# PantoMatrix/PantoMatrix

Hardware: NVIDIA H100
Metric: motion_frames_per_sec (higher is better)
Workload: dtype fp16x3 (two fp16 operand planes, 3 products, f32 accumulate)

## Files before the change

include/pm_emage.h:

```cpp
#ifndef PM_EMAGE_H
#define PM_EMAGE_H
#include <stdint.h>
#ifdef __cplusplus
extern "C" {
#endif

#define PM_ABI_VERSION 5
#define PM_FMT_F16 0x100
#define PM_TC_TILE_SHIFT 16
int pm_abi_version(void);
int pm_memset_async(void* ptr, int value, long long bytes, void* stream);
int pm_device_cc(void);

int pm_tapgemm_f32(const float* A, long long a_bs, int lda, int batch, int rows_in, int cin,
                   const float* W, const float* bias, int taps, int stride, int pad,
                   int rows_out, int cout,
                   const float* residual, long long r_bs, int ldr,
                   int act, float slope,
                   float* out, long long o_bs, int ldo, void* stream);

int pm_tapgemm_tc(const uint16_t* A, long long a_ps, long long a_bs, int lda, int batch, int rows_in, int cin,
                  const uint16_t* W, long long w_ps, int w_rows, int ldw, int taps, int pad, int nsplit,
                  const float* bias, int rows_out, int cout,
                  const float* residual, long long r_bs, int ldr,
                  int act, int act_cols, float slope, float acc_scale,
                  float* out_f32, long long o_bs, int ldo,
                  uint16_t* out_bf16, long long ob_ps, long long ob_bs, int ldob, int out_nsplit,
                  const void* prefetch, long long prefetch_bytes, void* stream);

int pm_split_bf16(const float* x, long long x_bs, int ldx, int batch, int rows, int ch,
                  uint16_t* out, long long o_ps, long long o_bs, int ldo, int nsplit, void* stream);

int pm_wav_stem_f32(const float* audio, long long a_bs, long long a_ws, int batch, int windows, int n_samples,
                    const float* w1, const float* b1, const float* wd, const float* bd, int cout,
                    int ksize, int stride, int pad, int rows_out, float slope,
                    float* y1, float* sc,
                    uint16_t* planes, long long p_ps, int p_ld, int p_nsplit, void* stream);

int pm_add_layernorm_f32(const float* x, const float* r, const float* gamma, const float* beta,
                         float* out, long long rows, int ch, float eps,
                         uint16_t* planes, long long p_ps, int p_ld, int p_nsplit, void* stream);

int pm_attention_f32(const float* Q, int ldq, const float* K, int ldk, const float* V, int ldv,
                     float* O, int ldo, int batch, int heads, int tq, int tk, int head_dim,
                     uint16_t* planes, long long p_ps, int p_ld, int p_nsplit, void* stream);

int pm_attention_tc(const uint16_t* Q, long long q_ps, long long q_bs, int ldq, int q_cols, int q_col0,
                    const uint16_t* K, long long k_ps, long long k_bs, int ldk, int k_cols, int k_col0,
                    const uint16_t* V, long long v_ps, long long v_bs, int ldv, int v_cols, int v_col0,
                    float* O, int ldo, int batch, int heads, int tq, int tk, int head_dim,
                    uint16_t* planes, long long p_ps, int p_ld, int p_nsplit, void* stream);

int pm_add_rows_f32(const float* x, const float* pe, const float* spk, int first, int second,
                    float* out, int batch, int rows, int ch,
                    uint16_t* planes, long long p_ps, int p_ld, int p_nsplit, void* stream);
int pm_add2_f32(const float* a, const float* b, float* out, long long n, int ch,
                uint16_t* planes, long long p_ps, int p_ld, int p_nsplit, void* stream);
int pm_add2_strided_f32(const float* a, long long lda, const float* b, long long ldb, float* out, long long ldo,
                        long long rows, long long ch,
                        uint16_t* planes, long long p_ps, int p_ld, int p_nsplit, void* stream);

int pm_window_input_f32(const float* motion, const float* mask, const float* seed, const float* mask_embedding,
                        float* out, int batch, int total_len, int start, int win_len, int pre, int ch, long long seed_bs,
                        uint16_t* planes, long long p_ps, int p_ld, int p_nsplit, void* stream);

int pm_l2_argmin_f32(const float* z, long long rows, int rows_per_batch, long long z_bs,
                     const float* codebook, const float* e2, int n_codes, int e_dim, long long* index, void* stream);
int pm_l2_argmin_tc(const float* z, long long rows, int rows_per_batch, long long z_bs,
                    const float* codebook, const float* e2, int n_codes, int e_dim, long long* index, int max_ctas,
                    void* stream);
int pm_l2_argmin_simt_f32(const float* z, long long rows, int rows_per_batch, long long z_bs,
                          const float* codebook, const float* e2, int n_codes, int e_dim, long long* index, void* stream);
int pm_row_argmax_f32(const float* x, long long rows, int ch, int ldx, int rows_per_batch, long long x_bs,
                      long long* index, int* nonfinite, void* stream);
int pm_gather_rows_f32(const float* codebook, long long n_table, const long long* index, long long rows, int ch,
                       float* out, uint16_t* planes, long long p_ps, int p_ld, int p_nsplit, void* stream);
int pm_row_sqnorm_f32(const float* x, int rows, int ch, float* out, void* stream);

int pm_pose_compose_f32(const float* face, const float* upper, const float* hands, const float* lower,
                        float* expression, float* axis_angle, float* motion4inf, long long bt, void* stream);

int pm_global_trans_f32(const float* rec, int ld, int vel_off, const float* ref_trans, int ref_bs, float dt,
                        float* trans, int batch, int t, void* stream);

int pm_resample_poly_f32(const void* pcm, int is_int16, long long in_bs, int batch, long long n_in, int channels,
                         const float* bank, int up, int down, int taps, long long n_pre_remove,
                         float* out, long long out_bs, void* stream);

int pm_lstm_bidir_f32(const float* xproj, long long x_bs, int ldx, const float* whh,
                      float* y, long long y_bs, int ldy, unsigned int* barrier,
                      int batch, int t, int hidden, void* stream);
int pm_lstm_cond_f32(const float* spk, long long n_spk, int spk_dim, const long long* speaker_id,
// ... 11 lines not shown
```

pantomatrix_b200/csrc/pm_tapgemm_tc.cu:

```cuda
#include <cuda.h>
#include <stdio.h>
#include <stdlib.h>

#include <cstring>
#include "pm_common.cuh"
#include "../../include/pm_emage.h"


namespace {

constexpr int BM = 128;
constexpr int BK = 64;
constexpr int MMA_K = 16;
constexpr int A_TILE_BYTES = BM * BK * 2;
constexpr int PRODUCER_THREADS = 128;
constexpr int CONSUMER_THREADS = 256;
constexpr int NUM_THREADS = PRODUCER_THREADS + CONSUMER_THREADS;
constexpr int PRODUCER_REGS = 40, CONSUMER_REGS = 232;
static_assert(PRODUCER_THREADS * PRODUCER_REGS + CONSUMER_THREADS * CONSUMER_REGS == (65536 / NUM_THREADS & ~7) * NUM_THREADS,
              "the setmaxnreg split must use exactly the launch's register pool");
constexpr int STAMP_WARP = PRODUCER_THREADS / 32;
constexpr int MAX_STAGES = 8;
constexpr int RING_KB = 200;

struct TcParams {
  int taps, pad, nsplit, kblocks;
  int rows_out, cout, batch;
  int R, NB;
  int w_rows;
  const float* bias;
  const float* residual; long long r_bs; int ldr;
  int act, act_cols; float slope;
  float* out_f32; long long o_bs; int ldo;
  __nv_bfloat16* out_bf16; long long ob_ps, ob_bs; int ldob; int out_nsplit;
  int stages;
  const uint8_t* prefetch; long long prefetch_bytes;
  float acc_scale;
};

#ifdef PM_TC_TIMING
__device__ unsigned long long pm_tc_stamps[4096 * 8];
#define PM_STAMP(i)                                                                                              \
  do {                                                                                                           \
    if ((threadIdx.x & 31) == 0) {                                                                               \
      const unsigned cta_ = (blockIdx.z * gridDim.y + blockIdx.y) * gridDim.x + blockIdx.x;                      \
      if (cta_ < 4096) pm_tc_stamps[cta_ * 8 + (i)] = (unsigned long long)clock64();                             \
    }                                                                                                            \
  } while (0)
#else
#define PM_STAMP(i) do {} while (0)
#endif

#include "pm_tc_ptx.cuh"

template <int BN, bool F16>
__device__ __forceinline__ void mma_k16(float (&d)[BN / 2], uint64_t a, uint64_t b) {
  static_assert(BN == 64 || BN == 128, "64- or 128-column tiles (see pm_tapgemm_tc)");
  if constexpr (BN == 64) wgmma_m64n64k16<!F16>(d, a, b);
  else wgmma_m64n128k16<!F16>(d, a, b);
}

template <int BN, bool F16, int NSPLIT>
__device__ __forceinline__ void mma_kblock(float (&main)[BN / 2], float (&corr)[BN / 2], uint64_t a0, uint64_t w0) {
  constexpr uint64_t A_PL = A_TILE_BYTES >> 4, W_PL = (BN * BK * 2) >> 4, K_ST = (MMA_K * 2) >> 4;
  if constexpr (NSPLIT == 3) {
#pragma unroll
    for (int k = 0; k < BK / MMA_K; ++k) mma_k16<BN, F16>(corr, a0 + k * K_ST, w0 + 2 * W_PL + k * K_ST);
#pragma unroll
    for (int k = 0; k < BK / MMA_K; ++k) mma_k16<BN, F16>(corr, a0 + A_PL + k * K_ST, w0 + W_PL + k * K_ST);
#pragma unroll
    for (int k = 0; k < BK / MMA_K; ++k) mma_k16<BN, F16>(corr, a0 + 2 * A_PL + k * K_ST, w0 + k * K_ST);
  }
  if constexpr (NSPLIT >= 2) {
#pragma unroll
    for (int k = 0; k < BK / MMA_K; ++k) mma_k16<BN, F16>(corr, a0 + k * K_ST, w0 + W_PL + k * K_ST);
#pragma unroll
    for (int k = 0; k < BK / MMA_K; ++k) mma_k16<BN, F16>(corr, a0 + A_PL + k * K_ST, w0 + k * K_ST);
  }
#pragma unroll
  for (int k = 0; k < BK / MMA_K; ++k) mma_k16<BN, F16>(main, a0 + k * K_ST, w0 + k * K_ST);
}

template <int BN, bool F16, int NSPLIT>
__global__ void __launch_bounds__(NUM_THREADS, 1) tapgemm_tc_kernel(const __grid_constant__ CUtensorMap map_a,
                                                                  const __grid_constant__ CUtensorMap map_w,
                                                                  const TcParams p) {
  constexpr int W_TILE_BYTES = BN * BK * 2;
  constexpr int NACC = BN / 2;
  constexpr int ST = BN + 8;

  extern __shared__ __align__(1024) uint8_t smem_raw[];
  uint8_t* tiles = reinterpret_cast<uint8_t*>((reinterpret_cast<uintptr_t>(smem_raw) + 1023) & ~uintptr_t(1023));
  const int stage_bytes = p.nsplit * (A_TILE_BYTES + W_TILE_BYTES);
  const int ring_bytes = p.stages * stage_bytes > BM * ST * 4 ? p.stages * stage_bytes : BM * ST * 4;
  uint64_t* bars = reinterpret_cast<uint64_t*>(tiles + ring_bytes);
  uint64_t* full_bar = bars;
  uint64_t* empty_bar = bars + MAX_STAGES;

  const int warp = threadIdx.x >> 5, lane = threadIdx.x & 31;
  if (warp == STAMP_WARP) PM_STAMP(0);
  const int l0 = blockIdx.x * p.R;
  const int n0 = blockIdx.y * BN;
  const int b0 = blockIdx.z * p.NB;
  const int n_iter = p.taps * p.kblocks;

  if (threadIdx.x == 0) {
    asm volatile("prefetch.tensormap [%0];" ::"l"(&map_a) : "memory");
    asm volatile("prefetch.tensormap [%0];" ::"l"(&map_w) : "memory");
    for (int s = 0; s < p.stages; ++s) {
      mbar_init(smem_u32(&full_bar[s]), 1);
      mbar_init(smem_u32(&empty_bar[s]), 2);
    }
    asm volatile("fence.mbarrier_init.release.cluster;" ::: "memory");
  }
  __syncthreads();
  if (warp == STAMP_WARP) PM_STAMP(1);

  if (warp < PRODUCER_THREADS / 32) {
    setmaxnreg_dec<PRODUCER_REGS>();
    if (warp == 1 && lane == 0 && p.prefetch) {
      const long long ncta = (long long)gridDim.x * gridDim.y * gridDim.z;
      const long long cta = ((long long)blockIdx.z * gridDim.y + blockIdx.y) * gridDim.x + blockIdx.x;
      long long share = ((p.prefetch_bytes + ncta - 1) / ncta + 127) & ~127LL;
      long long off = cta * share;
      long long end = off + share < p.prefetch_bytes ? off + share : p.prefetch_bytes;
      end &= ~15LL;
      for (; off < end; off += 16384) {
        const uint32_t n = (uint32_t)(end - off < 16384 ? end - off : 16384);
        asm volatile("cp.async.bulk.prefetch.L2.global [%0], %1;" ::"l"(p.prefetch + off), "r"(n) : "memory");
      }
    }
    if (warp != 0) return;
    const uint32_t tx = (uint32_t)stage_bytes;
    int s = 0, tap = 0, kb = 0;
    uint32_t ph = 0;
    for (int it = 0; it < n_iter; ++it) {
      mbar_wait_fast(smem_u32(&empty_bar[s]), ph ^ 1u);
      if (elect_one()) {
        const uint32_t bar = smem_u32(&full_bar[s]);
        uint8_t* st = tiles + (size_t)s * stage_bytes;
        mbar_expect_tx(bar, tx);
        for (int pl = 0; pl < p.nsplit; ++pl) {
          tma_load_4d(smem_u32(st + pl * A_TILE_BYTES), &map_a, bar, kb * BK, l0 + tap - p.pad, b0, pl);
          tma_load_3d(smem_u32(st + p.nsplit * A_TILE_BYTES + pl * W_TILE_BYTES), &map_w, bar, kb * BK, tap * p.w_rows + n0, pl);
        }
      }
      __syncwarp();
      if (++s == p.stages) { s = 0; ph ^= 1u; }
      if (++kb == p.kblocks) { kb = 0; ++tap; }
    }
    return;
  }

  setmaxnreg_inc<CONSUMER_REGS>();
  const int ct = threadIdx.x - PRODUCER_THREADS;
  const int wg = ct >> 7;
  float acc0[NACC], acc1[NACC], accc[NACC];
#pragma unroll
  for (int i = 0; i < NACC; ++i) { acc0[i] = 0.f; acc1[i] = 0.f; accc[i] = 0.f; }
  {
    const uint32_t tiles_u32 = smem_u32(tiles);
    int s = 0;
    uint32_t ph = 0;
    int prev = -1;
    auto kblock = [&](float (&main)[NACC]) {
      mbar_wait_fast(smem_u32(&full_bar[s]), ph);
      if (prev < 0 && warp == STAMP_WARP) PM_STAMP(2);
      const uint32_t a_base = tiles_u32 + (uint32_t)s * (uint32_t)stage_bytes + (uint32_t)wg * (64 * 128);
      const uint32_t w_base = tiles_u32 + (uint32_t)s * (uint32_t)stage_bytes + (uint32_t)(NSPLIT * A_TILE_BYTES);
      wgmma_fence();
      mma_kblock<BN, F16, NSPLIT>(main, accc, gmma_desc(GMMA_DESC_K_SW128, a_base), gmma_desc(GMMA_DESC_K_SW128, w_base));
      wgmma_commit();
      wgmma_wait<1>();
      if (prev >= 0 && ct % 128 == 0) mbar_arrive(smem_u32(&empty_bar[prev]));
      prev = s;
      if (++s == p.stages) { s = 0; ph ^= 1u; }
    };
    int it = 0;
    for (; it + 1 < n_iter; it += 2) {
      kblock(acc0);
      kblock(acc1);
    }
    if (it < n_iter) kblock(acc0);
    if (warp == STAMP_WARP) PM_STAMP(3);
    wgmma_wait<0>();
    if (warp == STAMP_WARP) PM_STAMP(4);
    wgmma_fence_regs(acc0);
    wgmma_fence_regs(acc1);
    wgmma_fence_regs(accc);
  }
  named_bar_sync(1, CONSUMER_THREADS);
  {
    const int wq = warp & 3, t4 = lane & 3;
    const int r0 = wg * 64 + wq * 16 + (lane >> 2);
    float* stg = reinterpret_cast<float*>(tiles);
#pragma unroll
    for (int i = 0; i < NACC / 4; ++i) {
      const int c = 8 * i + 2 * t4;
#pragma unroll
      for (int h = 0; h < 2; ++h) {
        float v0 = acc0[4 * i + 2 * h] + acc1[4 * i + 2 * h];
        float v1 = acc0[4 * i + 2 * h + 1] + acc1[4 * i + 2 * h + 1];
        v0 += accc[4 * i + 2 * h];
        v1 += accc[4 * i + 2 * h + 1];
        if constexpr (F16) { v0 *= p.acc_scale; v1 *= p.acc_scale; }
        *reinterpret_cast<float2*>(stg + (r0 + 8 * h) * ST + c) = make_float2(v0, v1);
      }
    }
  }
  named_bar_sync(1, CONSUMER_THREADS);

  const bool vec_f = p.out_f32 && ((p.ldo & 3) == 0) && ((reinterpret_cast<uintptr_t>(p.out_f32) & 15) == 0) && ((p.o_bs & 3) == 0);
  const bool vec_r = p.residual && ((p.ldr & 3) == 0) && ((reinterpret_cast<uintptr_t>(p.residual) & 15) == 0) && ((p.r_bs & 3) == 0);
  const bool vec_b = p.out_bf16 && ((p.ldob & 3) == 0) && ((reinterpret_cast<uintptr_t>(p.out_bf16) & 7) == 0) &&
                     ((p.ob_bs & 3) == 0) && ((p.ob_ps & 3) == 0);
  const bool all_vec = (!p.out_f32 || vec_f) && (!p.residual || vec_r) && (!p.out_bf16 || vec_b);
  const float act_slope = p.act == PM_ACT_NONE ? 1.f : (p.act == PM_ACT_RELU ? 0.f : p.slope);
  const int r_shift = 31 - __clz(p.R);
  constexpr int C4 = BN / 4;
  const float* stg = reinterpret_cast<const float*>(tiles);
#pragma unroll 1
  for (int item = ct; item < BM * C4; item += CONSUMER_THREADS) {
    const int rt = item / C4, c = (item % C4) * 4;
    const int b = b0 + (rt >> r_shift), l = l0 + (rt & (p.R - 1));
    const int n = n0 + c;
    if (b >= p.batch || l >= p.rows_out || n >= p.cout) continue;
    const float4 x4 = *reinterpret_cast<const float4*>(stg + rt * ST + c);
    const long long of = (long long)b * p.o_bs + (long long)l * p.ldo;
    const long long orr = (long long)b * p.r_bs + (long long)l * p.ldr;
    const PmPlanes P{p.out_bf16 ? p.out_bf16 + (long long)b * p.ob_bs + (long long)l * p.ldob : nullptr,
                     p.ob_ps, p.ldob, p.out_nsplit};
    if (all_vec && n + 4 <= p.cout) {
      float4 x = x4;
      if (p.bias) { x.x += __ldg(p.bias + n); x.y += __ldg(p.bias + n + 1); x.z += __ldg(p.bias + n + 2); x.w += __ldg(p.bias + n + 3); }
      if (p.residual) {
        const float4 t = *reinterpret_cast<const float4*>(p.residual + orr + n);
        x.x += t.x; x.y += t.y; x.z += t.z; x.w += t.w;
      }
      x.x = x.x < 0.f ? (n < p.act_cols ? act_slope : 1.f) * x.x : x.x;
      x.y = x.y < 0.f ? (n + 1 < p.act_cols ? act_slope : 1.f) * x.y : x.y;
      x.z = x.z < 0.f ? (n + 2 < p.act_cols ? act_slope : 1.f) * x.z : x.z;
      x.w = x.w < 0.f ? (n + 3 < p.act_cols ? act_slope : 1.f) * x.w : x.w;
      if (p.out_f32) *reinterpret_cast<float4*>(p.out_f32 + of + n) = x;
      if (P.ptr) pm_store_planes4_t<F16>(P, 0, n, x);
    } else {
      const float xs[4] = {x4.x, x4.y, x4.z, x4.w};
#pragma unroll
      for (int k = 0; k < 4; ++k) {
        if (n + k >= p.cout) break;
        float y = xs[k];
        if (p.bias) y += __ldg(p.bias + n + k);
        if (p.residual) y += p.residual[orr + n + k];
        y = y < 0.f ? (n + k < p.act_cols ? act_slope : 1.f) * y : y;
        if (p.out_f32) p.out_f32[of + n + k] = y;
        if (P.ptr) pm_store_planes_t<F16>(P, 0, n + k, y);
      }
    }
  }
  if (warp == STAMP_WARP) PM_STAMP(5);
#ifdef PM_TC_TIMING
  named_bar_sync(1, CONSUMER_THREADS);
#endif
  if (warp == STAMP_WARP) PM_STAMP(6);
}

template <bool VEC, bool F16>
__global__ void __launch_bounds__(256) split_bf16_kernel(const float* __restrict__ x, long long x_bs, int ldx, int rows,
                                                         int ch, __nv_bfloat16* __restrict__ out, long long o_ps,
                                                         long long o_bs, int ldo, int nsplit) {
  const int b = blockIdx.y;
  const float* __restrict__ xb = x + (long long)b * x_bs;
  __nv_bfloat16* __restrict__ ob = out + (long long)b * o_bs;
  if (VEC) {
    const int ch4 = ch >> 2;
    const long long total = (long long)rows * ch4;
    for (long long i = (long long)blockIdx.x * blockDim.x + threadIdx.x; i < total; i += (long long)gridDim.x * blockDim.x) {
      const int r = (int)(i / ch4), c4 = (int)(i - (long long)r * ch4);
      const float4 v = *reinterpret_cast<const float4*>(xb + (long long)r * ldx + 4 * c4);
      const PmPlanes P{ob, o_ps, ldo, nsplit};
      pm_store_planes4_t<F16>(P, r, 4 * c4, v);
    }
  } else {
    const long long total = (long long)rows * ch;
    for (long long i = (long long)blockIdx.x * blockDim.x + threadIdx.x; i < total; i += (long long)gridDim.x * blockDim.x) {
      const int r = (int)(i / ch), c = (int)(i - (long long)r * ch);
      const PmPlanes P{ob, o_ps, ldo, nsplit};
      pm_store_planes_t<F16>(P, r, c, xb[(long long)r * ldx + c]);
    }
  }
}

template <int BN, bool F16, int NSPLIT>
int launch(const CUtensorMap& ma, const CUtensorMap& mw, TcParams& p, dim3 grid, cudaStream_t st) {
  const int stage_bytes = p.nsplit * (A_TILE_BYTES + BN * BK * 2);
  int stages = RING_KB * 1024 / stage_bytes;
  if (stages > MAX_STAGES) stages = MAX_STAGES;
  if (stages < 2) return PM_EUNSUPPORTED;
  p.stages = stages;
  const int staging = BM * (BN + 8) * 4;
  const size_t ring = (size_t)stages * stage_bytes > (size_t)staging ? (size_t)stages * stage_bytes : (size_t)staging;
  const size_t smem = ring + 1024  + 2 * MAX_STAGES * sizeof(uint64_t);
  static unsigned long long configured = 0;
  if (pm_first_use_on_device(configured)) {
    cudaError_t e = cudaFuncSetAttribute(tapgemm_tc_kernel<BN, F16, NSPLIT>, cudaFuncAttributeMaxDynamicSharedMemorySize, 227 * 1024);
    if (e != cudaSuccess) { configured = 0; return (int)e; }
  }
  tapgemm_tc_kernel<BN, F16, NSPLIT><<<grid, NUM_THREADS, smem, st>>>(ma, mw, p);
  PM_LAUNCH_CHECK();
}

template <int BN>
int launch_fmt(const CUtensorMap& ma, const CUtensorMap& mw, TcParams& p, dim3 grid, cudaStream_t st, bool f16) {
  if (f16) {
    if (p.nsplit == 1) return launch<BN, true, 1>(ma, mw, p, grid, st);
    if (p.nsplit == 2) return launch<BN, true, 2>(ma, mw, p, grid, st);
    return launch<BN, true, 3>(ma, mw, p, grid, st);
  }
  if (p.nsplit == 1) return launch<BN, false, 1>(ma, mw, p, grid, st);
  if (p.nsplit == 2) return launch<BN, false, 2>(ma, mw, p, grid, st);
  return launch<BN, false, 3>(ma, mw, p, grid, st);
}

int pick_bn(long long row_tiles, int cout, int w_rows, int sms) {
  if (cout <= 64 || w_rows % 128) return 64;
  const long long waves64 = (row_tiles * pm_cdiv(cout, 64) + sms - 1) / sms;
  const long long waves128 = (row_tiles * pm_cdiv(cout, 128) + sms - 1) / sms;
  return waves128 * 14 <= waves64 * 10 ? 128 : 64;
}

}

extern "C" int pm_tapgemm_tc(const uint16_t* A, long long a_ps, long long a_bs, int lda, int batch, int rows_in, int cin,
                             const uint16_t* W, long long w_ps, int w_rows, int ldw, int taps, int pad, int nsplit,
                             const float* bias, int rows_out, int cout,
                             const float* residual, long long r_bs, int ldr,
                             int act, int act_cols, float slope, float acc_scale,
                             float* out_f32, long long o_bs, int ldo,
                             uint16_t* out_bf16, long long ob_ps, long long ob_bs, int ldob, int out_nsplit,
                             const void* prefetch, long long prefetch_bytes, void* stream) {
  PM_REQUIRE(A && W && (out_f32 || out_bf16));
  const int tile = (nsplit >> PM_TC_TILE_SHIFT) & 0xff;
  PM_TAKE_FMT(nsplit, f16);
  PM_TAKE_FMT(out_nsplit, out_f16);
  PM_REQUIRE(!out_bf16 || out_f16 == f16);
  PM_REQUIRE(f16 || acc_scale == 1.0f);
  PM_REQUIRE(!prefetch || (prefetch_bytes >= 0 && (reinterpret_cast<uintptr_t>(prefetch) & 15) == 0));
  PM_REQUIRE(batch > 0 && rows_in > 0 && rows_out > 0 && cin > 0 && cout > 0 && taps > 0);
  PM_REQUIRE(nsplit >= 1 && nsplit <= 3 && (!out_bf16 || (out_nsplit >= 1 && out_nsplit <= 3)));
  PM_REQUIRE(act >= PM_ACT_NONE && act <= PM_ACT_LEAKY);
  PM_REQUIRE((reinterpret_cast<uintptr_t>(A) & 15) == 0 && (reinterpret_cast<uintptr_t>(W) & 15) == 0);
  PM_REQUIRE((lda & 7) == 0 && (ldw & 7) == 0 && lda >= cin && ldw >= cin && w_rows >= cout);
  PM_REQUIRE(batch == 1 || (a_bs & 7) == 0);
  PM_REQUIRE(nsplit == 1 || ((a_ps & 7) == 0 && (w_ps & 7) == 0));
  PM_REQUIRE(!out_f32 || ldo >= cout);
  PM_REQUIRE(!out_bf16 || ldob >= cout);
  PM_REQUIRE(!residual || ldr >= cout);

  int R = 128;
  if (rows_out <= 64 && batch > 1) { R = 16; while (R < rows_out) R <<= 1; }
  const int NB = 128 / R;
  PM_REQUIRE(tile <= 2 && w_rows % 64 == 0 && (tile != 2 || w_rows % 128 == 0));
  int BNsel = tile == 1 ? 64 : 128;
  if (tile == 0) {
    int dev = 0, sms = 0;
    cudaError_t e = cudaGetDevice(&dev);
    if (e == cudaSuccess) e = cudaDeviceGetAttribute(&sms, cudaDevAttrMultiProcessorCount, dev);
    if (e != cudaSuccess) return (int)e;
    BNsel = pick_bn((long long)pm_cdiv(rows_out, R) * pm_cdiv(batch, NB), cout, w_rows, sms);
  }

  TcParams p;
  p.taps = taps; p.pad = pad; p.nsplit = nsplit; p.kblocks = (cin + BK - 1) / BK;
  p.rows_out = rows_out; p.cout = cout; p.batch = batch; p.R = R; p.NB = NB; p.w_rows = w_rows;
  p.bias = bias; p.residual = residual; p.r_bs = r_bs; p.ldr = ldr;
  p.act = act; p.act_cols = act_cols <= 0 ? cout : act_cols; p.slope = slope;
  p.out_f32 = out_f32; p.o_bs = o_bs; p.ldo = ldo;
  p.out_bf16 = reinterpret_cast<__nv_bfloat16*>(out_bf16); p.ob_ps = ob_ps; p.ob_bs = ob_bs; p.ldob = ldob;
  p.out_nsplit = out_bf16 ? out_nsplit : 0;
  p.stages = 0;
  p.prefetch = static_cast<const uint8_t*>(prefetch);
  p.prefetch_bytes = prefetch ? prefetch_bytes : 0;
  p.acc_scale = acc_scale;
  CUtensorMap ma, mw;
  {
    const long long bs_el = batch > 1 ? a_bs : (long long)rows_in * lda;
    const long long ps_el = nsplit > 1 ? a_ps : bs_el * batch;
    cuuint64_t dims[4] = {(cuuint64_t)cin, (cuuint64_t)rows_in, (cuuint64_t)batch, (cuuint64_t)nsplit};
    cuuint64_t strides[3] = {(cuuint64_t)lda * 2, (cuuint64_t)bs_el * 2, (cuuint64_t)ps_el * 2};
    cuuint32_t box[4] = {(cuuint32_t)BK, (cuuint32_t)R, (cuuint32_t)NB, 1};
    if (!encode_map(&ma, A, 4, dims, strides, box, f16)) return PM_EBADARG;
  }
  {
    const long long ps_el = nsplit > 1 ? w_ps : (long long)taps * w_rows * ldw;
    cuuint64_t dims[3] = {(cuuint64_t)cin, (cuuint64_t)taps * w_rows, (cuuint64_t)nsplit};
    cuuint64_t strides[2] = {(cuuint64_t)ldw * 2, (cuuint64_t)ps_el * 2};
    cuuint32_t box[3] = {(cuuint32_t)BK, (cuuint32_t)BNsel, 1};
    if (!encode_map(&mw, W, 3, dims, strides, box, f16)) return PM_EBADARG;
  }
  dim3 grid(pm_cdiv(rows_out, R), pm_cdiv(cout, BNsel), pm_cdiv(batch, NB));
  PM_REQUIRE(grid.z <= 65535 && grid.y <= 65535);
  const cudaStream_t st = (cudaStream_t)stream;
  if (BNsel == 128) return launch_fmt<128>(ma, mw, p, grid, st, f16);
  return launch_fmt<64>(ma, mw, p, grid, st, f16);
}

#ifdef PM_TC_TIMING
extern "C" int pm_tc_timing_reset() {
  cudaError_t e = cudaDeviceSynchronize();
  if (e != cudaSuccess) return (int)e;
  void* d = nullptr;
  e = cudaGetSymbolAddress(&d, pm_tc_stamps);
  if (e != cudaSuccess) return (int)e;
  return (int)cudaMemset(d, 0, sizeof(unsigned long long) * 4096 * 8);
}
extern "C" int pm_tc_timing_read(unsigned long long* host) {
  cudaError_t e = cudaDeviceSynchronize();
  if (e != cudaSuccess) return (int)e;
  return (int)cudaMemcpyFromSymbol(host, pm_tc_stamps, sizeof(unsigned long long) * 4096 * 8);
}
#endif

extern "C" int pm_split_bf16(const float* x, long long x_bs, int ldx, int batch, int rows, int ch,
                             uint16_t* out, long long o_ps, long long o_bs, int ldo, int nsplit, void* stream) {
  PM_TAKE_FMT(nsplit, f16);
  PM_REQUIRE(x && out && batch >= 0 && rows >= 0 && ch > 0 && ldx >= ch && ldo >= ch && nsplit >= 1 && nsplit <= 3);
  if ((long long)batch * rows == 0) return PM_OK;
  PM_REQUIRE(batch <= 65535);
  const bool vec = (ch & 3) == 0 && (ldx & 3) == 0 && (x_bs & 3) == 0 && (ldo & 3) == 0 && (o_bs & 3) == 0 &&
                   (o_ps & 3) == 0 && (reinterpret_cast<uintptr_t>(x) & 15) == 0 && (reinterpret_cast<uintptr_t>(out) & 7) == 0;
  const long long work = (long long)rows * (vec ? ch / 4 : ch);
  long long gx = (work + 255) / 256;
  const long long cap = batch >= 132 * 4 ? 1 : (132 * 8 + batch - 1) / batch;
  if (gx > cap) gx = cap;
  dim3 grid((unsigned)gx, batch);
  __nv_bfloat16* o = reinterpret_cast<__nv_bfloat16*>(out);
  cudaStream_t st = (cudaStream_t)stream;
  if (f16) {
    if (vec) split_bf16_kernel<true, true><<<grid, 256, 0, st>>>(x, x_bs, ldx, rows, ch, o, o_ps, o_bs, ldo, nsplit);
    else split_bf16_kernel<false, true><<<grid, 256, 0, st>>>(x, x_bs, ldx, rows, ch, o, o_ps, o_bs, ldo, nsplit);
  } else {
    if (vec) split_bf16_kernel<true, false><<<grid, 256, 0, st>>>(x, x_bs, ldx, rows, ch, o, o_ps, o_bs, ldo, nsplit);
    else split_bf16_kernel<false, false><<<grid, 256, 0, st>>>(x, x_bs, ldx, rows, ch, o, o_ps, o_bs, ldo, nsplit);
  }
  PM_LAUNCH_CHECK();
}
```

pantomatrix_b200/ops.py:

```python
from __future__ import annotations

import math

import torch

from . import _lib

ACT_NONE, ACT_RELU, ACT_LEAKY = 0, 1, 2
ROW_NONE, ROW_PE, ROW_SPK = 0, 1, 2

launch_count = 0

FMT_F16 = 0x100
TC_TILE_SHIFT = 16
F16_ACT_SCALE = 64.0
_PLANE_DTYPE = torch.bfloat16


def set_plane_format(name: str) -> None:
    global _PLANE_DTYPE
    _PLANE_DTYPE = {"bf16": torch.bfloat16, "fp16": torch.float16}[name]


def plane_format() -> str:
    return "fp16" if _PLANE_DTYPE == torch.float16 else "bf16"


def _fmt_bit(t) -> int:
    return FMT_F16 if t.dtype == torch.float16 else 0


def _stream() -> int:
    return torch.cuda.current_stream().cuda_stream


def _ptr(t) -> int | None:
    return None if t is None else t.data_ptr()


def _chk(t: torch.Tensor, dtype=torch.float32):
    if not t.is_cuda:
        raise _lib.PmError("pantomatrix_b200 ops need CUDA tensors (no CPU fallback)")
    if t.dtype != dtype:
        raise _lib.PmError(f"expected {dtype}, got {t.dtype}")
    if t.dim() and t.stride(-1) != 1 and t.shape[-1] != 1:
        raise _lib.PmError("innermost dimension must be contiguous")
    return t


def _call(name, *args):
    global launch_count
    launch_count += 1
    _lib.call(name, *args)


def _bs_ld(t: torch.Tensor):
    return (t.stride(0) if t.shape[0] > 1 else t.shape[1] * t.stride(1)), t.stride(1)


def tapgemm(a, w, bias, *, rows_out=None, stride=1, pad=0, act=ACT_NONE, slope=0.0, residual=None, out=None):
    _chk(a), _chk(w)
    batch, rows_in, cin = a.shape
    taps, cout, cin_w = w.shape
    assert cin_w == cin and w.is_contiguous(), (w.shape, a.shape)
    if rows_out is None:
        rows_out = (rows_in + 2 * pad - taps) // stride + 1
    if out is None:
        out = torch.empty(batch, rows_out, cout, device=a.device, dtype=torch.float32)
    else:
        assert out.shape == (batch, rows_out, cout), (out.shape, (batch, rows_out, cout))
    _chk(out)
    if residual is not None:
        _chk(residual)
        assert residual.shape == out.shape
    if (taps == 1 and pad == 0 and stride == 1 and batch > 1 and a.stride(0) == rows_in * a.stride(1)
            and out.stride(0) == rows_out * out.stride(1)
            and (residual is None or residual.stride(0) == rows_out * residual.stride(1))):
        a = a.reshape(1, batch * rows_in, cin) if a.is_contiguous() else a.as_strided(
            (1, batch * rows_in, cin), (0, a.stride(1), 1), a.storage_offset())
        flat = lambda t: t.as_strided((1, batch * rows_out, cout), (0, t.stride(1), 1), t.storage_offset())
        out_v = flat(out)
        res_v = flat(residual) if residual is not None else None
        batch_k, rows_in_k, rows_out_k = 1, batch * rows_in, batch * rows_out
    else:
        out_v, res_v, batch_k, rows_in_k, rows_out_k = out, residual, batch, rows_in, rows_out
    a_bs, lda = _bs_ld(a)
    o_bs, ldo = _bs_ld(out_v)
    r_bs, ldr = _bs_ld(res_v) if res_v is not None else (0, 0)
    _call("pm_tapgemm_f32", a.data_ptr(), a_bs, lda, batch_k, rows_in_k, cin,
          w.data_ptr(), _ptr(bias), taps, stride, pad, rows_out_k, cout,
          _ptr(res_v), r_bs, ldr, act, float(slope), out_v.data_ptr(), o_bs, ldo, _stream())
    return out


def wav_stem(audio, a_bs, a_ws, batch, windows, n_samples, w1, b1, wd, bd, *, stride, pad, slope, offset=0, nsplit=0):
    _chk(audio)
    cout, ks = w1.shape
# ... 261 lines not shown
    expression = torch.empty(bs, t, 100, device=device, dtype=torch.float32)
    axis_angle = torch.empty(bs, t, 165, device=device, dtype=torch.float32)
    motion4inf = torch.empty(bs, t, 337, device=device, dtype=torch.float32)
    _call("pm_pose_compose_f32", _ptr(face), _ptr(upper), _ptr(hands), _ptr(lower), expression.data_ptr(),
          axis_angle.data_ptr(), motion4inf.data_ptr(), bs * t, _stream())
    return expression, axis_angle, motion4inf


def global_trans(rec, ref_trans, dt, vel_off=54):
    _chk(rec), _chk(ref_trans)
    assert rec.is_contiguous()
    bs, t, ld = rec.shape
    assert ref_trans.shape == (bs, 3)
    trans = torch.empty(bs, t, 3, device=rec.device, dtype=torch.float32)
    _call("pm_global_trans_f32", rec.data_ptr(), ld, vel_off, ref_trans.data_ptr(), ref_trans.stride(0), float(dt),
          trans.data_ptr(), bs, t, _stream())
    return trans




def _round_up(x, m):
    return (x + m - 1) // m * m


class Planes:
    __slots__ = ("t", "rows", "ch", "slack")

    def __init__(self, t, rows, ch, slack=0):
        self.t, self.rows, self.ch, self.slack = t, rows, ch, slack

    def flat(self):
        ns, b, r, ld = self.t.shape
        assert self.t.stride(1) == r * self.t.stride(2)
        return Planes(self.t.as_strided((ns, 1, b * r, ld), (self.t.stride(0), b * r * self.t.stride(2), self.t.stride(2), 1),
                                        self.t.storage_offset()), b * r, self.ch, self.slack)

    @property
    def nsplit(self):
        return self.t.shape[0]

    @property
    def batch(self):
        return self.t.shape[1]


def split_bf16(x, nsplit, slack_rows=0):
    _chk(x)
    batch, rows, ch = x.shape
    pl = _new_planes(nsplit, (batch, rows), ch, x.device, slack_rows)
    x_bs, ldx = _bs_ld(x)
    _call("pm_split_bf16", x.data_ptr(), x_bs, ldx, batch, rows, ch, pl.t.data_ptr(), pl.t.stride(0), pl.t.stride(1),
          pl.t.stride(2), nsplit | _fmt_bit(pl.t), _stream())
    return pl


class PackedW:
    __slots__ = ("t", "taps", "cout", "cin", "w_rows", "ldw", "acc_scale")

    def __init__(self, w, nsplit):
        taps, cout, cin = w.shape
        bn = 64 if cout <= 64 else 128
        self.taps, self.cout, self.cin = taps, cout, cin
        self.w_rows, self.ldw = _round_up(cout, bn), _round_up(cin, 8)
        full = torch.zeros(taps, self.w_rows, self.ldw, device=w.device, dtype=torch.float32)
        full[:, :cout, :cin] = w
        self.acc_scale = 1.0
        if _PLANE_DTYPE == torch.float16:
            m = float(full.abs().max())
            if m > 0.0 and math.isfinite(m):
                k = math.floor(math.log2(32768.0 / m))
                full = full * (2.0 ** k)
                self.acc_scale = 2.0 ** -k
            self.acc_scale /= F16_ACT_SCALE
        planes, rem = [], full
        for _ in range(nsplit):
            p = rem.to(_PLANE_DTYPE)
            planes.append(p)
            rem = rem - p.float()
        self.t = torch.stack(planes).contiguous()


def tapgemm_tc(a: Planes, w: PackedW, bias, *, rows_in=None, rows_out, pad=0, act=ACT_NONE, act_cols=0, slope=0.0,
               residual=None, want_f32=True, out_nsplit=0, out=None, a_view=None, out_slack=0, prefetch=None, tile=0):
    t = a.t
    nsplit, batch = t.shape[0], t.shape[1]
    assert nsplit == w.t.shape[0] and t.dtype == w.t.dtype, "A and W must use the same split and plane format"
    fmt = _fmt_bit(t)
    rows_a, cin, lda = (a.rows, a.ch, t.stride(2)) if a_view is None else a_view
    if rows_in is not None:
        rows_a = rows_in
    assert cin == w.cin, (cin, w.cin)
    assert tile in (0, 64, 128), tile
    cout = w.cout
    dev = t.device
    out_f = None
    if want_f32:
        out_f = out if out is not None else torch.empty(batch, rows_out, cout, device=dev, dtype=torch.float32)
        assert out_f.shape == (batch, rows_out, cout)
    o_bs, ldo = _bs_ld(out_f) if out_f is not None else (0, 0)
    out_p = None
    if out_nsplit:
        out_p = _new_planes(out_nsplit, (batch, rows_out), cout, dev, out_slack, dtype=t.dtype)
    r_bs, ldr = _bs_ld(residual) if residual is not None else (0, 0)
    if residual is not None:
        _chk(residual)
        assert residual.shape == (batch, rows_out, cout)
    _call("pm_tapgemm_tc", t.data_ptr(), t.stride(0), t.stride(1), lda, batch, rows_a, cin,
          w.t.data_ptr(), w.t.stride(0), w.w_rows, w.ldw, w.taps, pad, nsplit | fmt | (tile // 64) << TC_TILE_SHIFT,
          _ptr(bias), rows_out, cout, _ptr(residual), r_bs, ldr, act, act_cols, float(slope), float(w.acc_scale),
          _ptr(out_f), o_bs, ldo,
          None if out_p is None else out_p.t.data_ptr(), 0 if out_p is None else out_p.t.stride(0),
          0 if out_p is None else out_p.t.stride(1), 0 if out_p is None else out_p.t.stride(2),
          out_nsplit | (fmt if out_nsplit else 0),
          None if prefetch is None else prefetch.data_ptr(),
          0 if prefetch is None else prefetch.numel() * prefetch.element_size(), _stream())
    return out_f, out_p




def lstm_bidir(xproj, whh, barrier, hidden):
    _chk(xproj), _chk(whh)
    assert xproj.is_contiguous() and whh.is_contiguous() and whh.shape == (2, 4 * hidden, hidden)
    batch, t, w = xproj.shape
    assert w == 8 * hidden
    y = torch.empty(batch, t, 2 * hidden, device=xproj.device, dtype=torch.float32)
    _call("pm_lstm_bidir_f32", xproj.data_ptr(), xproj.stride(0), xproj.stride(1), whh.data_ptr(), y.data_ptr(),
          y.stride(0), y.stride(1), barrier.data_ptr(), batch, t, hidden, _stream())
    return y


def rot6d_to_aa(rot6d, slot, n_sel):
    _chk(rot6d)
    assert rot6d.is_contiguous() and rot6d.shape[-1] == n_sel * 6
    rows = rot6d.numel() // (n_sel * 6)
    out = torch.empty(*rot6d.shape[:-1], 165, device=rot6d.device, dtype=torch.float32)
    _call("pm_rot6d_to_aa_f32", rot6d.data_ptr(), rows, n_sel, slot.data_ptr(), out.data_ptr(), _stream())
    return out


def softmax2_mix(sel, c1, c2, out=None):
    _chk(sel), _chk(c1), _chk(c2)
    assert sel.is_contiguous() and c1.is_contiguous() and c2.is_contiguous() and sel.shape[-1] == 2
    ch = c1.shape[-1]
    rows = c1.numel() // ch
    if out is None:
        out = torch.empty_like(c1)
    _call("pm_softmax2_mix_f32", sel.data_ptr(), c1.data_ptr(), c2.data_ptr(), out.data_ptr(), rows, ch, out.stride(-2), _stream())
    return out
```

Before: 248,300.

## Make tapgemm TC kernel persistent with per-warp register epilogue staging

Measured after the change: 251,200, median of 6. 1.2% higher.

```diff
diff --git a/include/pm_emage.h b/include/pm_emage.h
--- a/include/pm_emage.h
+++ b/include/pm_emage.h
@@ -8,6 +8,7 @@
 #define PM_ABI_VERSION 5
 #define PM_FMT_F16 0x100
 #define PM_TC_TILE_SHIFT 16
+#define PM_TC_GRID_SHIFT 24
 int pm_abi_version(void);
 int pm_memset_async(void* ptr, int value, long long bytes, void* stream);
 int pm_device_cc(void);
diff --git a/pantomatrix_b200/csrc/pm_tapgemm_tc.cu b/pantomatrix_b200/csrc/pm_tapgemm_tc.cu
--- a/pantomatrix_b200/csrc/pm_tapgemm_tc.cu
+++ b/pantomatrix_b200/csrc/pm_tapgemm_tc.cu
@@ -21,12 +21,16 @@
               "the setmaxnreg split must use exactly the launch's register pool");
 constexpr int STAMP_WARP = PRODUCER_THREADS / 32;
 constexpr int MAX_STAGES = 8;
+constexpr int EPI_COLS = 32, EPI_LD = 40;
+constexpr int EPI_WARP_FLOATS = 16 * EPI_LD + 128;
+constexpr int EPI_BYTES = (CONSUMER_THREADS / 32) * EPI_WARP_FLOATS * 4;
 constexpr int RING_KB = 200;
 
 struct TcParams {
   int taps, pad, nsplit, kblocks;
   int rows_out, cout, batch;
   int R, NB;
+  int tiles_x, tiles_y, tiles;
   int w_rows;
   const float* bias;
   const float* residual; long long r_bs; int ldr;
@@ -40,15 +44,14 @@
 
 #ifdef PM_TC_TIMING
 __device__ unsigned long long pm_tc_stamps[4096 * 8];
-#define PM_STAMP(i)                                                                                              \
+#define PM_STAMP_VAL(tile, i, v)                                                                                 \
   do {                                                                                                           \
-    if ((threadIdx.x & 31) == 0) {                                                                               \
-      const unsigned cta_ = (blockIdx.z * gridDim.y + blockIdx.y) * gridDim.x + blockIdx.x;                      \
-      if (cta_ < 4096) pm_tc_stamps[cta_ * 8 + (i)] = (unsigned long long)clock64();                             \
-    }                                                                                                            \
+    if ((threadIdx.x & 31) == 0 && (tile) < 4096) pm_tc_stamps[(tile) * 8 + (i)] = (unsigned long long)(v);      \
   } while (0)
+#define PM_STAMP(tile, i) PM_STAMP_VAL(tile, i, clock64())
 #else
-#define PM_STAMP(i) do {} while (0)
+#define PM_STAMP_VAL(tile, i, v) do {} while (0)
+#define PM_STAMP(tile, i) do {} while (0)
 #endif
 
 #include "pm_tc_ptx.cuh"
@@ -87,21 +90,20 @@
                                                                   const TcParams p) {
   constexpr int W_TILE_BYTES = BN * BK * 2;
   constexpr int NACC = BN / 2;
-  constexpr int ST = BN + 8;
 
   extern __shared__ __align__(1024) uint8_t smem_raw[];
   uint8_t* tiles = reinterpret_cast<uint8_t*>((reinterpret_cast<uintptr_t>(smem_raw) + 1023) & ~uintptr_t(1023));
   const int stage_bytes = p.nsplit * (A_TILE_BYTES + W_TILE_BYTES);
-  const int ring_bytes = p.stages * stage_bytes > BM * ST * 4 ? p.stages * stage_bytes : BM * ST * 4;
-  uint64_t* bars = reinterpret_cast<uint64_t*>(tiles + ring_bytes);
+  uint64_t* bars = reinterpret_cast<uint64_t*>(tiles + p.stages * stage_bytes);
   uint64_t* full_bar = bars;
   uint64_t* empty_bar = bars + MAX_STAGES;
+  float* epi_stage = reinterpret_cast<float*>(bars + 2 * MAX_STAGES);
 
   const int warp = threadIdx.x >> 5, lane = threadIdx.x & 31;
-  if (warp == STAMP_WARP) PM_STAMP(0);
-  const int l0 = blockIdx.x * p.R;
-  const int n0 = blockIdx.y * BN;
-  const int b0 = blockIdx.z * p.NB;
+#ifdef PM_TC_TIMING
+  const long long t_entry = clock64();
+  long long t_ready = 0;
+#endif
   const int n_iter = p.taps * p.kblocks;
 
   if (threadIdx.x == 0) {
@@ -114,13 +116,15 @@
     asm volatile("fence.mbarrier_init.release.cluster;" ::: "memory");
   }
   __syncthreads();
-  if (warp == STAMP_WARP) PM_STAMP(1);
+#ifdef PM_TC_TIMING
+  t_ready = clock64();
+#endif
 
   if (warp < PRODUCER_THREADS / 32) {
     setmaxnreg_dec<PRODUCER_REGS>();
     if (warp == 1 && lane == 0 && p.prefetch) {
-      const long long ncta = (long long)gridDim.x * gridDim.y * gridDim.z;
-      const long long cta = ((long long)blockIdx.z * gridDim.y + blockIdx.y) * gridDim.x + blockIdx.x;
+      const long long ncta = gridDim.x;
+      const long long cta = blockIdx.x;
       long long share = ((p.prefetch_bytes + ncta - 1) / ncta + 127) & ~127LL;
       long long off = cta * share;
       long long end = off + share < p.prefetch_bytes ? off + share : p.prefetch_bytes;
@@ -132,22 +136,28 @@
     }
     if (warp != 0) return;
     const uint32_t tx = (uint32_t)stage_bytes;
-    int s = 0, tap = 0, kb = 0;
+    int s = 0;
     uint32_t ph = 0;
-    for (int it = 0; it < n_iter; ++it) {
-      mbar_wait_fast(smem_u32(&empty_bar[s]), ph ^ 1u);
-      if (elect_one()) {
-        const uint32_t bar = smem_u32(&full_bar[s]);
-        uint8_t* st = tiles + (size_t)s * stage_bytes;
-        mbar_expect_tx(bar, tx);
-        for (int pl = 0; pl < p.nsplit; ++pl) {
-          tma_load_4d(smem_u32(st + pl * A_TILE_BYTES), &map_a, bar, kb * BK, l0 + tap - p.pad, b0, pl);
-          tma_load_3d(smem_u32(st + p.nsplit * A_TILE_BYTES + pl * W_TILE_BYTES), &map_w, bar, kb * BK, tap * p.w_rows + n0, pl);
+    for (int tile = blockIdx.x; tile < p.tiles; tile += gridDim.x) {
+      const int l0 = (tile % p.tiles_x) * p.R;
+      const int n0 = (tile / p.tiles_x % p.tiles_y) * BN;
+      const int b0 = tile / p.tiles_x / p.tiles_y * p.NB;
+      int tap = 0, kb = 0;
+      for (int it = 0; it < n_iter; ++it) {
+        mbar_wait_fast(smem_u32(&empty_bar[s]), ph ^ 1u);
+        if (elect_one()) {
+          const uint32_t bar = smem_u32(&full_bar[s]);
+          uint8_t* st = tiles + (size_t)s * stage_bytes;
+          mbar_expect_tx(bar, tx);
+          for (int pl = 0; pl < p.nsplit; ++pl) {
+            tma_load_4d(smem_u32(st + pl * A_TILE_BYTES), &map_a, bar, kb * BK, l0 + tap - p.pad, b0, pl);
+            tma_load_3d(smem_u32(st + p.nsplit * A_TILE_BYTES + pl * W_TILE_BYTES), &map_w, bar, kb * BK, tap * p.w_rows + n0, pl);
+          }
         }
+        __syncwarp();
+        if (++s == p.stages) { s = 0; ph ^= 1u; }
+        if (++kb == p.kblocks) { kb = 0; ++tap; }
       }
-      __syncwarp();
-      if (++s == p.stages) { s = 0; ph ^= 1u; }
-      if (++kb == p.kblocks) { kb = 0; ++tap; }
     }
     return;
   }
@@ -155,61 +165,7 @@
   setmaxnreg_inc<CONSUMER_REGS>();
   const int ct = threadIdx.x - PRODUCER_THREADS;
   const int wg = ct >> 7;
-  float acc0[NACC], acc1[NACC], accc[NACC];
-#pragma unroll
-  for (int i = 0; i < NACC; ++i) { acc0[i] = 0.f; acc1[i] = 0.f; accc[i] = 0.f; }
-  {
-    const uint32_t tiles_u32 = smem_u32(tiles);
-    int s = 0;
-    uint32_t ph = 0;
-    int prev = -1;
-    auto kblock = [&](float (&main)[NACC]) {
-      mbar_wait_fast(smem_u32(&full_bar[s]), ph);
-      if (prev < 0 && warp == STAMP_WARP) PM_STAMP(2);
-      const uint32_t a_base = tiles_u32 + (uint32_t)s * (uint32_t)stage_bytes + (uint32_t)wg * (64 * 128);
-      const uint32_t w_base = tiles_u32 + (uint32_t)s * (uint32_t)stage_bytes + (uint32_t)(NSPLIT * A_TILE_BYTES);
-      wgmma_fence();
-      mma_kblock<BN, F16, NSPLIT>(main, accc, gmma_desc(GMMA_DESC_K_SW128, a_base), gmma_desc(GMMA_DESC_K_SW128, w_base));
-      wgmma_commit();
-      wgmma_wait<1>();
-      if (prev >= 0 && ct % 128 == 0) mbar_arrive(smem_u32(&empty_bar[prev]));
-      prev = s;
-      if (++s == p.stages) { s = 0; ph ^= 1u; }
-    };
-    int it = 0;
-    for (; it + 1 < n_iter; it += 2) {
-      kblock(acc0);
-      kblock(acc1);
-    }
-    if (it < n_iter) kblock(acc0);
-    if (warp == STAMP_WARP) PM_STAMP(3);
-    wgmma_wait<0>();
-    if (warp == STAMP_WARP) PM_STAMP(4);
-    wgmma_fence_regs(acc0);
-    wgmma_fence_regs(acc1);
-    wgmma_fence_regs(accc);
-  }
-  named_bar_sync(1, CONSUMER_THREADS);
-  {
-    const int wq = warp & 3, t4 = lane & 3;
-    const int r0 = wg * 64 + wq * 16 + (lane >> 2);
-    float* stg = reinterpret_cast<float*>(tiles);
-#pragma unroll
-    for (int i = 0; i < NACC / 4; ++i) {
-      const int c = 8 * i + 2 * t4;
-#pragma unroll
-      for (int h = 0; h < 2; ++h) {
-        float v0 = acc0[4 * i + 2 * h] + acc1[4 * i + 2 * h];
-        float v1 = acc0[4 * i + 2 * h + 1] + acc1[4 * i + 2 * h + 1];
-        v0 += accc[4 * i + 2 * h];
-        v1 += accc[4 * i + 2 * h + 1];
-        if constexpr (F16) { v0 *= p.acc_scale; v1 *= p.acc_scale; }
-        *reinterpret_cast<float2*>(stg + (r0 + 8 * h) * ST + c) = make_float2(v0, v1);
-      }
-    }
-  }
-  named_bar_sync(1, CONSUMER_THREADS);
-
+  const uint32_t tiles_u32 = smem_u32(tiles);
   const bool vec_f = p.out_f32 && ((p.ldo & 3) == 0) && ((reinterpret_cast<uintptr_t>(p.out_f32) & 15) == 0) && ((p.o_bs & 3) == 0);
   const bool vec_r = p.residual && ((p.ldr & 3) == 0) && ((reinterpret_cast<uintptr_t>(p.residual) & 15) == 0) && ((p.r_bs & 3) == 0);
   const bool vec_b = p.out_bf16 && ((p.ldob & 3) == 0) && ((reinterpret_cast<uintptr_t>(p.out_bf16) & 7) == 0) &&
@@ -217,51 +173,122 @@
   const bool all_vec = (!p.out_f32 || vec_f) && (!p.residual || vec_r) && (!p.out_bf16 || vec_b);
   const float act_slope = p.act == PM_ACT_NONE ? 1.f : (p.act == PM_ACT_RELU ? 0.f : p.slope);
   const int r_shift = 31 - __clz(p.R);
-  constexpr int C4 = BN / 4;
-  const float* stg = reinterpret_cast<const float*>(tiles);
+  int s = 0;
+  uint32_t ph = 0;
 #pragma unroll 1
-  for (int item = ct; item < BM * C4; item += CONSUMER_THREADS) {
-    const int rt = item / C4, c = (item % C4) * 4;
-    const int b = b0 + (rt >> r_shift), l = l0 + (rt & (p.R - 1));
-    const int n = n0 + c;
-    if (b >= p.batch || l >= p.rows_out || n >= p.cout) continue;
-    const float4 x4 = *reinterpret_cast<const float4*>(stg + rt * ST + c);
-    const long long of = (long long)b * p.o_bs + (long long)l * p.ldo;
-    const long long orr = (long long)b * p.r_bs + (long long)l * p.ldr;
-    const PmPlanes P{p.out_bf16 ? p.out_bf16 + (long long)b * p.ob_bs + (long long)l * p.ldob : nullptr,
-                     p.ob_ps, p.ldob, p.out_nsplit};
-    if (all_vec && n + 4 <= p.cout) {
-      float4 x = x4;
-      if (p.bias) { x.x += __ldg(p.bias + n); x.y += __ldg(p.bias + n + 1); x.z += __ldg(p.bias + n + 2); x.w += __ldg(p.bias + n + 3); }
-      if (p.residual) {
-        const float4 t = *reinterpret_cast<const float4*>(p.residual + orr + n);
-        x.x += t.x; x.y += t.y; x.z += t.z; x.w += t.w;
+  for (int tile = blockIdx.x; tile < p.tiles; tile += gridDim.x) {
+    const int l0 = (tile % p.tiles_x) * p.R;
+    const int n0 = (tile / p.tiles_x % p.tiles_y) * BN;
+    const int b0 = tile / p.tiles_x / p.tiles_y * p.NB;
+    if (warp == STAMP_WARP) { PM_STAMP_VAL(tile, 0, t_entry); PM_STAMP_VAL(tile, 1, t_ready); PM_STAMP_VAL(tile, 7, blockIdx.x + 1); }
+    float acc0[NACC], acc1[NACC], accc[NACC];
+#pragma unroll
+    for (int i = 0; i < NACC; ++i) { acc0[i] = 0.f; acc1[i] = 0.f; accc[i] = 0.f; }
+    {
+      int prev = -1;
+      auto kblock = [&](float (&main)[NACC]) {
+        mbar_wait_fast(smem_u32(&full_bar[s]), ph);
+        if (prev < 0 && warp == STAMP_WARP) PM_STAMP(tile, 2);
+        const uint32_t a_base = tiles_u32 + (uint32_t)s * (uint32_t)stage_bytes + (uint32_t)wg * (64 * 128);
+        const uint32_t w_base = tiles_u32 + (uint32_t)s * (uint32_t)stage_bytes + (uint32_t)(NSPLIT * A_TILE_BYTES);
+        wgmma_fence();
+        mma_kblock<BN, F16, NSPLIT>(main, accc, gmma_desc(GMMA_DESC_K_SW128, a_base), gmma_desc(GMMA_DESC_K_SW128, w_base));
+        wgmma_commit();
+        wgmma_wait<1>();
+        if (prev >= 0 && ct % 128 == 0) mbar_arrive(smem_u32(&empty_bar[prev]));
+        prev = s;
+        if (++s == p.stages) { s = 0; ph ^= 1u; }
+      };
+      int it = 0;
+      for (; it + 1 < n_iter; it += 2) {
+        kblock(acc0);
+        kblock(acc1);
       }
-      x.x = x.x < 0.f ? (n < p.act_cols ? act_slope : 1.f) * x.x : x.x;
-      x.y = x.y < 0.f ? (n + 1 < p.act_cols ? act_slope : 1.f) * x.y : x.y;
-      x.z = x.z < 0.f ? (n + 2 < p.act_cols ? act_slope : 1.f) * x.z : x.z;
-      x.w = x.w < 0.f ? (n + 3 < p.act_cols ? act_slope : 1.f) * x.w : x.w;
-      if (p.out_f32) *reinterpret_cast<float4*>(p.out_f32 + of + n) = x;
-      if (P.ptr) pm_store_planes4_t<F16>(P, 0, n, x);
-    } else {
-      const float xs[4] = {x4.x, x4.y, x4.z, x4.w};
-#pragma unroll
-      for (int k = 0; k < 4; ++k) {
-        if (n + k >= p.cout) break;
-        float y = xs[k];
-        if (p.bias) y += __ldg(p.bias + n + k);
-        if (p.residual) y += p.residual[orr + n + k];
-        y = y < 0.f ? (n + k < p.act_cols ? act_slope : 1.f) * y : y;
-        if (p.out_f32) p.out_f32[of + n + k] = y;
-        if (P.ptr) pm_store_planes_t<F16>(P, 0, n + k, y);
+      if (it < n_iter) kblock(acc0);
+      if (warp == STAMP_WARP) PM_STAMP(tile, 3);
+      wgmma_wait<0>();
+      if (warp == STAMP_WARP) PM_STAMP(tile, 4);
+      if (ct % 128 == 0) mbar_arrive(smem_u32(&empty_bar[prev]));
+      wgmma_fence_regs(acc0);
+      wgmma_fence_regs(acc1);
+      wgmma_fence_regs(accc);
+    }
+#pragma unroll
+    for (int i = 0; i < NACC; ++i) {
+      acc0[i] = (acc0[i] + acc1[i]) + accc[i];
+      if constexpr (F16) acc0[i] *= p.acc_scale;
+    }
+
+    float* stg = epi_stage + (warp - STAMP_WARP) * EPI_WARP_FLOATS;
+    float* stg_bias = stg + 16 * EPI_LD;
+    const int wrow = wg * 64 + (warp & 3) * 16;
+    if (p.bias) {
+      __syncwarp();
+      for (int c = lane; c < BN; c += 32) stg_bias[c] = n0 + c < p.cout ? __ldg(p.bias + n0 + c) : 0.f;
+    }
+#pragma unroll 1
+    for (int cc = 0; cc < BN / EPI_COLS; ++cc) {
+      const int n_chunk = n0 + cc * EPI_COLS;
+      if (n_chunk >= p.cout) break;
+      __syncwarp();
+#pragma unroll
+      for (int i = 0; i < NACC / 4; ++i) {
+        if (i / (EPI_COLS / 8) != cc) continue;
+        const int c = 8 * (i % (EPI_COLS / 8)) + 2 * (lane & 3);
+#pragma unroll
+        for (int h = 0; h < 2; ++h)
+          *reinterpret_cast<float2*>(stg + ((lane >> 2) + 8 * h) * EPI_LD + c) = make_float2(acc0[4 * i + 2 * h], acc0[4 * i + 2 * h + 1]);
       }
-    }
-  }
-  if (warp == STAMP_WARP) PM_STAMP(5);
+      __syncwarp();
+#pragma unroll 1
+      for (int k = 0; k < 16 * EPI_COLS / 4 / 32; ++k) {
+        const int rw = (lane >> 3) + 4 * k, c = (lane & 7) * 4;
+        const int rt = wrow + rw;
+        const int b = b0 + (rt >> r_shift), l = l0 + (rt & (p.R - 1));
+        const int n = n_chunk + c;
+        if (b >= p.batch || l >= p.rows_out || n >= p.cout) continue;
+        const float4 x4 = *reinterpret_cast<const float4*>(stg + rw * EPI_LD + c);
+        const long long of = (long long)b * p.o_bs + (long long)l * p.ldo;
+        const long long orr = (long long)b * p.r_bs + (long long)l * p.ldr;
+        const PmPlanes P{p.out_bf16 ? p.out_bf16 + (long long)b * p.ob_bs + (long long)l * p.ldob : nullptr,
+                         p.ob_ps, p.ldob, p.out_nsplit};
+        if (all_vec && n + 4 <= p.cout) {
+          float4 x = x4;
+          if (p.bias) {
+            const float4 bv = *reinterpret_cast<const float4*>(stg_bias + cc * EPI_COLS + c);
+            x.x += bv.x; x.y += bv.y; x.z += bv.z; x.w += bv.w;
+          }
+          if (p.residual) {
+            const float4 t = *reinterpret_cast<const float4*>(p.residual + orr + n);
+            x.x += t.x; x.y += t.y; x.z += t.z; x.w += t.w;
+          }
+          x.x = x.x < 0.f ? (n < p.act_cols ? act_slope : 1.f) * x.x : x.x;
+          x.y = x.y < 0.f ? (n + 1 < p.act_cols ? act_slope : 1.f) * x.y : x.y;
+          x.z = x.z < 0.f ? (n + 2 < p.act_cols ? act_slope : 1.f) * x.z : x.z;
+          x.w = x.w < 0.f ? (n + 3 < p.act_cols ? act_slope : 1.f) * x.w : x.w;
+          if (p.out_f32) *reinterpret_cast<float4*>(p.out_f32 + of + n) = x;
+          if (P.ptr) pm_store_planes4_t<F16>(P, 0, n, x);
+        } else {
+          const float xs[4] = {x4.x, x4.y, x4.z, x4.w};
+#pragma unroll
+          for (int e = 0; e < 4; ++e) {
+            if (n + e >= p.cout) break;
+            float y = xs[e];
+            if (p.bias) y += stg_bias[cc * EPI_COLS + c + e];
+            if (p.residual) y += p.residual[orr + n + e];
+            y = y < 0.f ? (n + e < p.act_cols ? act_slope : 1.f) * y : y;
+            if (p.out_f32) p.out_f32[of + n + e] = y;
+            if (P.ptr) pm_store_planes_t<F16>(P, 0, n + e, y);
+          }
+        }
+      }
+    }
+    if (warp == STAMP_WARP) PM_STAMP(tile, 5);
 #ifdef PM_TC_TIMING
-  named_bar_sync(1, CONSUMER_THREADS);
-#endif
-  if (warp == STAMP_WARP) PM_STAMP(6);
+    named_bar_sync(1, CONSUMER_THREADS);
+#endif
+    if (warp == STAMP_WARP) PM_STAMP(tile, 6);
+  }
 }
 
 template <bool VEC, bool F16>
@@ -297,9 +324,8 @@
   if (stages > MAX_STAGES) stages = MAX_STAGES;
   if (stages < 2) return PM_EUNSUPPORTED;
   p.stages = stages;
-  const int staging = BM * (BN + 8) * 4;
-  const size_t ring = (size_t)stages * stage_bytes > (size_t)staging ? (size_t)stages * stage_bytes : (size_t)staging;
-  const size_t smem = ring + 1024  + 2 * MAX_STAGES * sizeof(uint64_t);
+  const size_t smem = (size_t)stages * stage_bytes + 1024  + 2 * MAX_STAGES * sizeof(uint64_t) + EPI_BYTES;
+  if (smem > 227 * 1024) return PM_EUNSUPPORTED;
   static unsigned long long configured = 0;
   if (pm_first_use_on_device(configured)) {
     cudaError_t e = cudaFuncSetAttribute(tapgemm_tc_kernel<BN, F16, NSPLIT>, cudaFuncAttributeMaxDynamicSharedMemorySize, 227 * 1024);
@@ -321,11 +347,22 @@
   return launch<BN, false, 3>(ma, mw, p, grid, st);
 }
 
+#ifndef PM_TC_BN_RATIO10
+#define PM_TC_BN_RATIO10 14
+#endif
 int pick_bn(long long row_tiles, int cout, int w_rows, int sms) {
   if (cout <= 64 || w_rows % 128) return 64;
   const long long waves64 = (row_tiles * pm_cdiv(cout, 64) + sms - 1) / sms;
   const long long waves128 = (row_tiles * pm_cdiv(cout, 128) + sms - 1) / sms;
-  return waves128 * 14 <= waves64 * 10 ? 128 : 64;
+  return waves128 * PM_TC_BN_RATIO10 <= waves64 * 10 ? 128 : 64;
+}
+
+#ifndef PM_TC_PERSIST_MIN_WAVES
+#define PM_TC_PERSIST_MIN_WAVES 2
+#endif
+long long pick_grid(long long tiles, int sms) {
+  const long long waves = (tiles + sms - 1) / sms;
+  return waves < PM_TC_PERSIST_MIN_WAVES ? tiles : sms;
 }
 
 }
@@ -340,6 +377,7 @@
                              const void* prefetch, long long prefetch_bytes, void* stream) {
   PM_REQUIRE(A && W && (out_f32 || out_bf16));
   const int tile = (nsplit >> PM_TC_TILE_SHIFT) & 0xff;
+  const int grid_cap = (nsplit >> PM_TC_GRID_SHIFT) & 0x7f;
   PM_TAKE_FMT(nsplit, f16);
   PM_TAKE_FMT(out_nsplit, out_f16);
   PM_REQUIRE(!out_bf16 || out_f16 == f16);
@@ -360,18 +398,23 @@
   if (rows_out <= 64 && batch > 1) { R = 16; while (R < rows_out) R <<= 1; }
   const int NB = 128 / R;
   PM_REQUIRE(tile <= 2 && w_rows % 64 == 0 && (tile != 2 || w_rows % 128 == 0));
-  int BNsel = tile == 1 ? 64 : 128;
-  if (tile == 0) {
-    int dev = 0, sms = 0;
+  int dev = 0, sms = 0;
+  {
     cudaError_t e = cudaGetDevice(&dev);
     if (e == cudaSuccess) e = cudaDeviceGetAttribute(&sms, cudaDevAttrMultiProcessorCount, dev);
     if (e != cudaSuccess) return (int)e;
-    BNsel = pick_bn((long long)pm_cdiv(rows_out, R) * pm_cdiv(batch, NB), cout, w_rows, sms);
-  }
+  }
+  const long long row_tiles = (long long)pm_cdiv(rows_out, R) * pm_cdiv(batch, NB);
+  const int BNsel = tile == 0 ? pick_bn(row_tiles, cout, w_rows, sms) : (tile == 1 ? 64 : 128);
+  const long long ntiles = row_tiles * pm_cdiv(cout, BNsel);
+  PM_REQUIRE(ntiles < (1LL << 31));
+  long long nctas = grid_cap == 0 ? pick_grid(ntiles, sms) : (grid_cap == 0x7f ? ntiles : grid_cap);
+  if (nctas > ntiles) nctas = ntiles;
 
   TcParams p;
   p.taps = taps; p.pad = pad; p.nsplit = nsplit; p.kblocks = (cin + BK - 1) / BK;
   p.rows_out = rows_out; p.cout = cout; p.batch = batch; p.R = R; p.NB = NB; p.w_rows = w_rows;
+  p.tiles_x = pm_cdiv(rows_out, R); p.tiles_y = pm_cdiv(cout, BNsel); p.tiles = (int)ntiles;
   p.bias = bias; p.residual = residual; p.r_bs = r_bs; p.ldr = ldr;
   p.act = act; p.act_cols = act_cols <= 0 ? cout : act_cols; p.slope = slope;
   p.out_f32 = out_f32; p.o_bs = o_bs; p.ldo = ldo;
@@ -397,8 +440,7 @@
     cuuint32_t box[3] = {(cuuint32_t)BK, (cuuint32_t)BNsel, 1};
     if (!encode_map(&mw, W, 3, dims, strides, box, f16)) return PM_EBADARG;
   }
-  dim3 grid(pm_cdiv(rows_out, R), pm_cdiv(cout, BNsel), pm_cdiv(batch, NB));
-  PM_REQUIRE(grid.z <= 65535 && grid.y <= 65535);
+  const dim3 grid((unsigned)nctas);
   const cudaStream_t st = (cudaStream_t)stream;
   if (BNsel == 128) return launch_fmt<128>(ma, mw, p, grid, st, f16);
   return launch_fmt<64>(ma, mw, p, grid, st, f16);
diff --git a/pantomatrix_b200/ops.py b/pantomatrix_b200/ops.py
--- a/pantomatrix_b200/ops.py
+++ b/pantomatrix_b200/ops.py
@@ -13,6 +13,7 @@
 
 FMT_F16 = 0x100
 TC_TILE_SHIFT = 16
+TC_GRID_SHIFT = 24
 F16_ACT_SCALE = 64.0
 _PLANE_DTYPE = torch.bfloat16
 
@@ -440,7 +441,8 @@
 
 
 def tapgemm_tc(a: Planes, w: PackedW, bias, *, rows_in=None, rows_out, pad=0, act=ACT_NONE, act_cols=0, slope=0.0,
-               residual=None, want_f32=True, out_nsplit=0, out=None, a_view=None, out_slack=0, prefetch=None, tile=0):
+               residual=None, want_f32=True, out_nsplit=0, out=None, a_view=None, out_slack=0, prefetch=None, tile=0,
+               grid=0):
     t = a.t
     nsplit, batch = t.shape[0], t.shape[1]
     assert nsplit == w.t.shape[0] and t.dtype == w.t.dtype, "A and W must use the same split and plane format"
@@ -450,6 +452,7 @@
         rows_a = rows_in
     assert cin == w.cin, (cin, w.cin)
     assert tile in (0, 64, 128), tile
+    assert -1 <= grid <= 126, grid
     cout = w.cout
     dev = t.device
     out_f = None
@@ -465,7 +468,7 @@
         _chk(residual)
         assert residual.shape == (batch, rows_out, cout)
     _call("pm_tapgemm_tc", t.data_ptr(), t.stride(0), t.stride(1), lda, batch, rows_a, cin,
-          w.t.data_ptr(), w.t.stride(0), w.w_rows, w.ldw, w.taps, pad, nsplit | fmt | (tile // 64) << TC_TILE_SHIFT,
+          w.t.data_ptr(), w.t.stride(0), w.w_rows, w.ldw, w.taps, pad, nsplit | fmt | (tile // 64) << TC_TILE_SHIFT | (grid & 0x7f) << TC_GRID_SHIFT,
           _ptr(bias), rows_out, cout, _ptr(residual), r_bs, ldr, act, act_cols, float(slope), float(w.acc_scale),
           _ptr(out_f), o_bs, ldo,
           None if out_p is None else out_p.t.data_ptr(), 0 if out_p is None else out_p.t.stride(0),
```
